# SHI-Labs/SH-GAN

Measured on AMD Instinct MI355X. Metric: generator images/sec, higher is better.
Workload: dtype f32

## Files before the change

include/shgan_hip.h:

```cpp
#ifndef SHGAN_HIP_H
#define SHGAN_HIP_H
#include <stddef.h>
#include <stdint.h>
#ifdef __cplusplus
extern "C" {
#endif

#define SHG_OK 0
#define SHG_ERR_ARG (-1)
#define SHG_ERR_LAUNCH (-2)
#define SHG_ERR_UNSUPPORTED (-3)

int shg_abi_version(void);
const char* shg_last_error(void);
int shg_device_info(int dev, char* buf, int buflen);

int shg_upfirdn2d_out_size(int H, int W, int fh, int fw, int upx, int upy, int downx, int downy, int padx0, int padx1,
                           int pady0, int pady1, int* OH, int* OW);
int shg_upfirdn2d_f32(const float* x, const float* f, float* y, int N, int C, int H, int W, int fh, int fw, int upx, int upy,
                      int downx, int downy, int padx0, int padx1, int pady0, int pady1, int flip, float gain, void* stream);
int shg_upfirdn2d_strided(const void* x, const float* f, void* y, int dtype, int N, int C, int H, int W, const long* x_strides,
                          const long* y_strides, int fh, int fw, long f_stride_y, long f_stride_x, int upx, int upy, int downx, int downy,
                          int padx0, int padx1, int pady0, int pady1, int flip, float gain, void* stream);
int shg_upfirdn2d_epilogue_f32(const float* x, const float* f, float* y, int N, int C, int H, int W, int fh, int fw, int upx,
// ... 15 lines not shown
int shg_sum_partials_f32(const float* part, float* out, int N, int B, int K, void* stream);
int shg_scale_cast_f32_f16(const void* src, void* dst, long n, float gain, int to_half, void* stream);
int shg_planes_to_image_f32(const float* mid, const float* bias, float* y, int N, int C, int H, int W, int lo, int OH, int OW,
                            void* stream);

int shg_conv_weight_prep_f32(const float* w, float* wt, float* wscale, float* wsq, int O, int I, int KH, int KW, int OP,
                             int demod, float gain, int flip, void* stream);
int shg_conv2d_f32(const float* x, const float* wt, float* y, int NB, int I, int O, int OP, int H, int W, int kh, int kw,
                   int mode, int pad, int wgroups, long wstride, const float* in_scale, const float* out_scale,
                   const float* bias, const float* noise, int noise_mode, float noise_strength, int act, float alpha, float gain,
                   float clamp, const float* residual, int out_mode, void* workspace, size_t ws_bytes, void* stream);
size_t shg_conv2d_workspace_bytes(int NB, int I, int O, int H, int W, int kh, int kw, int mode, int pad, int wgroups);
int shg_conv_wino_chunk(void);
int shg_conv_weight_prep_wino_f32(const float* w, const float* wscale, float* wu, int O, int I, int OP, int flip, void* stream);
int shg_conv2d_wino_f32(const float* x, const float* wu, float* y, int NB, int I, int O, int OP, int H, int W,
                        const float* in_scale, const float* out_scale, const float* bias, const float* noise, int noise_mode,
                        float noise_strength, int act, float alpha, float gain, float clamp, const float* residual, void* stream);
size_t shg_conv2d_wino_workspace_bytes(int NB, int I, int O, int OP, int H, int W);
int shg_conv2d_wino_ws_f32(const float* x, const float* wu, float* y, int NB, int I, int O, int OP, int H, int W,
                           const float* in_scale, const float* out_scale, const float* bias, const float* noise, int noise_mode,
                           float noise_strength, int act, float alpha, float gain, float clamp, const float* residual, void* workspace,
                           size_t ws_bytes, void* stream);
long shg_conv_wino4_weight_elems(int OP, int I);
int shg_conv_weight_prep_wino4_f32(const float* w, const float* wscale, float* wu, int O, int I, int OP, int flip, void* stream);
int shg_conv2d_wino4_supported(int NB, int I, int O, int H, int W);
int shg_conv2d_wino4_f32(const float* x, const float* wu, float* y, int NB, int I, int O, int OP, int H, int W,
                         const float* in_scale, const float* out_scale, const float* bias, const float* noise, int noise_mode,
                         float noise_strength, int act, float alpha, float gain, float clamp, const float* residual, void* stream);
size_t shg_conv2d_wino4_workspace_bytes(int NB, int I, int O, int OP, int H, int W);
int shg_conv2d_wino4_ws_f32(const float* x, const float* wu, float* y, int NB, int I, int O, int OP, int H, int W,
                            const float* in_scale, const float* out_scale, const float* bias, const float* noise, int noise_mode,
                            float noise_strength, int act, float alpha, float gain, float clamp, const float* residual, void* workspace,
                            size_t ws_bytes, void* stream);
int shg_upfir_planar_f32(const float* mid, const float* f, float* y, int N, int C, int H, int W, int flip, float gain,
                         const float* scale, const float* bias, const float* noise, int noise_mode, float noise_strength,
                         int act, float alpha, float act_gain, float clamp, const float* residual, void* stream);
int shg_upfir_planar_sep_supported(int H, int W);
int shg_upfir_planar_sep_f32(const float* mid, const float* taps_host, float* y, int N, int C, int H, int W, int flip, float gain,
                             const float* scale, const float* bias, const float* noise, int noise_mode, float noise_strength,
                             int act, float alpha, float act_gain, float clamp, const float* residual, void* stream);
int shg_conv_weight_prep_up_poly_f32(const float* w, const float* wscale, float* wu_a, float* wu_b, int O, int I, int OP, int flip,
                                     void* stream);
int shg_conv2d_up_poly_supported(int NB, int I, int O, int H, int W);
int shg_conv2d_up_poly_f32(const float* x, const float* wt, const float* wu_a, const float* wu_b, float* y, int NB, int I, int O,
                           int OP, int H, int W, const float* in_scale, void* stream);
size_t shg_conv2d_up_poly_workspace_bytes(int NB, int I, int O, int OP, int H, int W);
int shg_conv2d_up_poly_ws_f32(const float* x, const float* wt, const float* wu_a, const float* wu_b, float* y, int NB, int I, int O,
                              int OP, int H, int W, const float* in_scale, void* workspace, size_t ws_bytes, void* stream);
int shg_fir_down_planar_f32(const float* x, const float* f, float* y, int N, int C, int H, int W, int PP, int flip, float gain,
                            void* stream);
int shg_fir_pad2_sep_supported(int H, int W, int PP);
int shg_fir_pad2_sep_f32(const float* x, const float* taps_host, float* y, int N, int C, int H, int W, int PP, int flip, float gain,
                         void* stream);
int shg_fir_resample2_sep_supported(int H, int W, int up);
int shg_fir_resample2_sep_f32(const float* x, const float* taps_host, float* y, int N, int C, int H, int W, int up, int flip, float gain,
                              void* stream);
int shg_conv_weight_prep_down_poly_f32(const float* w, const float* wscale, float* wu_a, float* wu_b, int O, int I, int OP, int flip,
                                       void* stream);
int shg_conv2d_down_poly_supported(int NB, int I, int O, int OH, int OW);
int shg_conv2d_down_poly_f32(const float* xp, const float* wu_a, const float* wu_b, float* y, int NB, int I, int O, int OP, int OH,
                             int OW, int PP, const float* in_scale, const float* bias, int act, float alpha, float gain,
                             float clamp, const float* residual, void* stream);
int shg_conv1x1_thin_in_f32(const float* x, const float* w, const float* bias, float* y, int N, int I, int O, int HW, float wgain,
                            int act, float alpha, float gain, float clamp, void* stream);
int shg_torgb_f32(const float* x, const float* w, const float* styles, const float* bias, const float* base_up, const float* f,
                  float* y, int N, int I, int O, int H, int W, void* stream);
// ... 169 lines not shown
```

sh-gan_amd/_lib.py:

```python
import ctypes
import os

import torch

_HERE = os.path.dirname(os.path.abspath(__file__))
LIB_PATH = os.path.join(_HERE, 'lib', 'libshgan_hip.so')
ABI_VERSION = 40

c_fp = ctypes.c_void_p
c_i = ctypes.c_int
c_f = ctypes.c_float
c_l = ctypes.c_long
c_pp = ctypes.POINTER(ctypes.c_void_p)



class DenseGroup(ctypes.Structure):
    _fields_ = [('x1', c_fp), ('x2', c_fp), ('w', c_fp), ('b', c_fp), ('y', c_fp),
                ('ld1', c_i), ('ld2', c_i), ('K1', c_i), ('K2', c_i), ('O', c_i), ('ldy', c_i),
                ('wgain', c_f), ('bgain', c_f)]


class StyleGroup(ctypes.Structure):
    _fields_ = [('styles', c_fp), ('wsq', c_fp), ('s_out', c_fp), ('dcoef', c_fp),
# ... 5 lines not shown
        (n, c_i) for n in ('I', 'H', 'W', 'x_ctot', 'x_coff', 'O', 'kh', 'kw', 'sh', 'sw', 'ph', 'pw', 'OH', 'OW', 'y_ctot', 'y_coff', 'splitk')]


_SIGS = {
    'shg_abi_version': [],
    'shg_device_info': [c_i, ctypes.c_char_p, c_i],
    'shg_upfirdn2d_out_size': [c_i] * 12 + [ctypes.POINTER(c_i), ctypes.POINTER(c_i)],
    'shg_upfirdn2d_f32': [c_fp, c_fp, c_fp] + [c_i] * 15 + [c_f, c_fp],
    'shg_upfirdn2d_strided': [c_fp, c_fp, c_fp, c_i, c_i, c_i, c_i, c_i, ctypes.POINTER(c_l), ctypes.POINTER(c_l), c_i, c_i, c_l, c_l] + [c_i] * 9
                             + [c_f, c_fp],
    'shg_upfirdn2d_epilogue_f32': [c_fp, c_fp, c_fp] + [c_i] * 15 + [c_f, c_fp, c_fp, c_fp, c_i, c_f, c_i, c_f, c_f, c_f, c_fp, c_fp],
    'shg_bias_act_f32': [c_fp, c_fp, c_fp, c_fp, c_fp, c_i, c_f, c_fp, c_i, c_i, c_i, c_i, c_f, c_f, c_f, c_fp],
    'shg_fma_f32': [c_fp, c_fp, c_fp, c_fp, c_l, c_fp],
    'shg_fma_bcast': [c_fp, c_fp, c_fp, c_fp, c_i] + [ctypes.POINTER(c_l)] * 4 + [c_i, c_fp],
    'shg_mul_reduce': [c_fp, c_fp, c_fp, c_i, c_i] + [ctypes.POINTER(c_l)] * 3 + [c_i, c_i, c_fp],
    'shg_scale_channels_f32': [c_fp, c_fp, c_fp, c_i, c_i, c_fp],
    'shg_sum_partials_f32': [c_fp, c_fp, c_i, c_i, c_i, c_fp],
    'shg_scale_cast_f32_f16': [c_fp, c_fp, c_l, c_f, c_i, c_fp],
    'shg_planes_to_image_f32': [c_fp, c_fp, c_fp, c_i, c_i, c_i, c_i, c_i, c_i, c_i, c_fp],
    'shg_conv_weight_prep_f32': [c_fp, c_fp, c_fp, c_fp, c_i, c_i, c_i, c_i, c_i, c_i, c_f, c_i, c_fp],
    'shg_conv2d_f32': [c_fp, c_fp, c_fp] + [c_i] * 11 + [c_l, c_fp, c_fp, c_fp, c_fp, c_i, c_f, c_i, c_f, c_f, c_f, c_fp, c_i,
                       c_fp, ctypes.c_size_t, c_fp],
    'shg_conv2d_workspace_bytes': [c_i] * 10,
    'shg_conv_wino_chunk': [],
    'shg_conv_weight_prep_wino_f32': [c_fp, c_fp, c_fp, c_i, c_i, c_i, c_i, c_fp],
    'shg_conv2d_wino_f32': [c_fp, c_fp, c_fp] + [c_i] * 6 + [c_fp, c_fp, c_fp, c_fp, c_i, c_f, c_i, c_f, c_f, c_f, c_fp, c_fp],
    'shg_conv2d_wino_ws_f32': [c_fp, c_fp, c_fp] + [c_i] * 6 + [c_fp, c_fp, c_fp, c_fp, c_i, c_f, c_i, c_f, c_f, c_f, c_fp, c_fp, ctypes.c_size_t, c_fp],
    'shg_conv2d_wino_workspace_bytes': [c_i] * 6,
    'shg_conv_wino4_weight_elems': [c_i, c_i],
    'shg_conv_weight_prep_wino4_f32': [c_fp, c_fp, c_fp, c_i, c_i, c_i, c_i, c_fp],
    'shg_conv2d_wino4_supported': [c_i] * 5,
    'shg_conv2d_wino4_f32': [c_fp, c_fp, c_fp] + [c_i] * 6 + [c_fp, c_fp, c_fp, c_fp, c_i, c_f, c_i, c_f, c_f, c_f, c_fp, c_fp],
    'shg_conv2d_wino4_ws_f32': [c_fp, c_fp, c_fp] + [c_i] * 6 + [c_fp, c_fp, c_fp, c_fp, c_i, c_f, c_i, c_f, c_f, c_f, c_fp, c_fp, ctypes.c_size_t, c_fp],
    'shg_conv2d_wino4_workspace_bytes': [c_i] * 6,
    'shg_upfir_planar_f32': [c_fp, c_fp, c_fp, c_i, c_i, c_i, c_i, c_i, c_f, c_fp, c_fp, c_fp, c_i, c_f, c_i, c_f, c_f, c_f, c_fp, c_fp],
    'shg_upfir_planar_sep_supported': [c_i, c_i],
    'shg_upfir_planar_sep_f32': [c_fp, ctypes.POINTER(c_f), c_fp, c_i, c_i, c_i, c_i, c_i, c_f, c_fp, c_fp, c_fp, c_i, c_f, c_i, c_f, c_f, c_f, c_fp, c_fp],
    'shg_conv1x1_thin_in_f32': [c_fp, c_fp, c_fp, c_fp, c_i, c_i, c_i, c_i, c_f, c_i, c_f, c_f, c_f, c_fp],
    'shg_torgb_f32': [c_fp, c_fp, c_fp, c_fp, c_fp, c_fp, c_fp, c_i, c_i, c_i, c_i, c_i, c_fp],
    'shg_dense_f32': [c_fp, c_fp, c_fp, c_fp, c_i, c_i, c_i, c_i, c_i, c_f, c_f, c_i, c_f, c_f, c_f, c_fp],
    'shg_demod_weight_f32': [c_fp, c_fp, c_fp, c_fp, c_i, c_i, c_i, c_i, c_fp],
    'shg_demod_weight_backward_f32': [c_fp, c_fp, c_fp, c_fp, c_fp, c_i, c_i, c_i, c_fp],
    'shg_style_factors_f32': [c_fp, c_fp, c_fp, c_fp, c_fp, c_i, c_i, c_i, c_i, c_fp],
    'shg_style_factors_backward_f32': [c_fp, c_fp, c_fp, c_fp, c_fp, c_fp, c_fp, c_fp, c_fp, c_i, c_i, c_i, c_i, c_fp],
    'shg_matmul_nn_f32': [c_fp, c_fp, c_fp, c_i, c_i, c_i, c_i, c_i, c_f, c_fp],
    'shg_matmul_tn_f32': [c_fp, c_fp, c_fp, c_fp, c_i, c_i, c_i, c_i, c_i, c_f, c_f, c_fp],
    'shg_normalize_2nd_moment_f32': [c_fp, c_fp, c_i, c_i, c_f, c_fp],
    'shg_modconv_style_prep_f32': [c_fp, c_i, c_fp, c_fp, c_fp, c_i, c_i, c_i, c_i, c_i, c_f, c_fp],
    'shg_dense_grouped_f32': [ctypes.POINTER(DenseGroup), c_i, c_i, c_fp],
    'shg_modconv_style_prep_grouped_f32': [ctypes.POINTER(StyleGroup), c_i, c_i, c_fp],
    'shg_shu_rfft2_shift_f32': [c_fp, c_l, c_fp, c_i, c_i, c_fp],
    'shg_bias_act_backward_f32': [c_fp, c_fp, c_fp, c_l, c_i, c_f, c_f, c_f, c_fp],
    'shg_conv2d_wgrad_workspace_bytes': [c_i] * 7,
    'shg_conv2d_wgrad_f32': [c_fp, c_fp, c_fp] + [c_i] * 11 + [c_fp, ctypes.c_size_t, c_fp],
    'shg_conv2d_wgrad_wino_supported': [c_i] * 8,
    'shg_conv2d_wgrad_wino_workspace_bytes': [c_i] * 5,
    'shg_conv2d_wgrad_wino_f32': [c_fp, c_fp, c_fp] + [c_i] * 5 + [c_fp, ctypes.c_size_t, c_fp],
    'shg_shu_spectral_f32': [c_fp] * 6 + [c_i] * 4 + [c_fp],
    'shg_shu_split_irfft2_f32': [c_fp, c_fp, c_pp, c_pp, ctypes.POINTER(c_l), c_i, c_i, c_i, c_i, c_fp],
    'shg_shu_split_adjoint_f32': [c_pp, ctypes.POINTER(c_l), c_pp, c_fp, c_i, c_i, c_fp],
    'shg_shu_rfft2_shift_n_f32': [c_fp, c_l, c_fp, c_i, c_i, c_i, c_fp],
    'shg_shu_spectral_n_f32': [c_fp] * 6 + [c_i] * 4 + [c_fp],
    'shg_shu_split_irfft2_n_f32': [c_fp, c_fp, c_pp, c_pp, ctypes.POINTER(c_l), c_i, c_i, c_i, c_i, c_i, ctypes.POINTER(c_i), c_i, c_fp],
    'shg_shu_split_adjoint_n_f32': [c_pp, ctypes.POINTER(c_l), c_pp, c_fp, c_i, c_i, c_i, ctypes.POINTER(c_i), c_i, c_fp],
    'shg_composite_u8': [c_fp, c_fp, c_fp, c_i, c_i, c_i, c_fp],
    'shg_assemble_input_f32': [c_fp, c_fp, c_fp, c_i, c_i, c_i, c_fp],
# ... 124 lines not shown
```

sh-gan_amd/csrc/conv_wino4.hip:

```cpp
#include "wino_common.h"
#include <stdlib.h>
#include <type_traits>

__device__ __attribute__((aligned(16))) float shg_wino4_zeros[64];

namespace wino4 {
constexpr int KC = 8, BO = 64, BT = 32, NPOS = 36, NW = 8, NT = NW * 64, NUNIT = 2 * NPOS;
constexpr int V_SZ = NPOS * KC * BT;
template <int TY, int TX>
struct Tile {
    static_assert(TY * TX == BT, "32 blocks per tile");
    static constexpr int PH = 4 * TY + 2, PW = 4 * TX + 8, PW4 = PW / 4, PATCH4 = PH * PW4;
    static constexpr int NPIECE = (PATCH4 + 63) / 64, RP = NPIECE * 256, R_SZ = KC * RP;
};
static_assert(2 * V_SZ >= NPOS * 16 * 32, "epilogue exchange buffer lives in the V region");
}

template <class T>
__device__ __forceinline__ void wino4_bt(const T (&d)[6], T (&o)[6]) {
    const T a = d[4] - 4.f * d[2], b = d[3] - 4.f * d[1], c = d[4] - d[2], e = 2.f * (d[3] - d[1]);
    o[0] = 4.f * d[0] - 5.f * d[2] + d[4];
    o[1] = a + b; o[2] = a - b;
    o[3] = c + e; o[4] = c - e;
    o[5] = 4.f * d[1] - 5.f * d[3] + d[5];
}
__device__ __forceinline__ void wino4_at(const float (&m)[6], float (&o)[4]) {
    float s12 = m[1] + m[2], d12 = m[1] - m[2], s34 = m[3] + m[4], d34 = m[3] - m[4];
    shg_opaque(s12); shg_opaque(d12); shg_opaque(s34); shg_opaque(d34);
    o[0] = m[0] + s12 + s34;
    o[1] = d12 + 2.f * d34;
    o[2] = s12 + 4.f * s34;
    o[3] = d12 + 8.f * d34 + m[5];
}

template <int TY, int TX>
__global__ __launch_bounds__(512, 2) void conv_wino4_kernel(const WinoParams p) {
    using namespace wino4;
    using T = Tile<TY, TX>;
    constexpr int PW = T::PW, PW4 = T::PW4, PATCH4 = T::PATCH4, RP = T::RP, R_SZ = T::R_SZ, NPIECE = T::NPIECE;
    __shared__ __attribute__((aligned(16))) float Vl[2 * V_SZ];
    __shared__ __attribute__((aligned(16))) float Rl[2 * R_SZ];

    const int tid = threadIdx.x;
    const int lane = tid & 63, wave = __builtin_amdgcn_readfirstlane(tid >> 6);
    const int l31 = lane & 31, half = lane >> 5;

    const int nwork = p.n_ttiles * p.n_otiles;
    const int work = shg_xcd_remap(blockIdx.x, nwork);
    const int otile = work / p.n_ttiles;
    const int ttile = work - otile * p.n_ttiles;
    const int txb = ttile % p.tiles_x;
    const int tyb = (ttile / p.tiles_x) % p.tiles_y;
    const int n = ttile / (p.tiles_x * p.tiles_y);
    const int oy0 = tyb * (4 * TY), ox0 = txb * (4 * TX);
    const int o0 = otile * BO;
    const int HW = p.H * p.W;
    const int c0 = blockIdx.y * p.cps, nch = min(p.cps, p.nchunk - c0), iend = min(p.I, (c0 + nch) * KC);

    const bool xformer = wave < 4;
    int roff[NPIECE];
#pragma unroll
    for (int j = 0; j < NPIECE; ++j) {
        const int q = j * 64 + lane;
        const int py = q / PW4, p4 = q - py * PW4;
        const int iy = oy0 - 1 + py, ix = ox0 - 4 + 4 * p4;
        const bool ok = q < PATCH4 && iy >= 0 && iy < p.H && ix >= 0 && ix + 3 < p.W;
        roff[j] = ok ? n * p.I * HW + iy * p.W + ix : -1;
    }
    auto dma_piece = [&](int c, int buf, int q, int j) __attribute__((always_inline)) {
        const int k = (wave - 4) * 2 + q;
        const int ch = (c0 + c) * KC + k;
        const bool chok = ch < iend;
        const float* src = (chok && roff[j] >= 0) ? p.x + ((long)roff[j] + (long)ch * HW) : shg_wino4_zeros;
        const unsigned lds = __builtin_amdgcn_readfirstlane(
// ... 23 lines not shown
        const float s1 = __builtin_bit_cast(float, __builtin_amdgcn_readlane(__builtin_bit_cast(int, ca < 64 ? scb[0] : scb[1]), ca & 63));
        return half ? s1 : s0;
    };
    auto tr_read = [&](int r, f32x4 (&w)[3], int buf) __attribute__((always_inline)) {
        const f32x4* rb = reinterpret_cast<const f32x4*>(rbase + buf * R_SZ + r * PW);
#pragma unroll
        for (int q = 0; q < 3; ++q) w[q] = rb[q];
    };
    auto tr_row = [&](int r, const f32x4 (&w)[3], float (&u)[6][6], float sc) __attribute__((always_inline)) {
        const float di[6] = {w[0][3] * sc, w[1][0] * sc, w[1][1] * sc, w[1][2] * sc, w[1][3] * sc, w[2][0] * sc};
        wino4_bt(di, u[r]);
    };
    auto tr_col = [&](int j, const float (&u)[6][6], int buf) __attribute__((always_inline)) {
        float* vb = vbase + buf * V_SZ + j * KC * BT;
        const float di[6] = {u[0][j], u[1][j], u[2][j], u[3][j], u[4][j], u[5][j]};
        float o[6];
        wino4_bt(di, o);
#pragma unroll
        for (int i = 0; i < 6; ++i) vb[i * 6 * KC * BT] = o[i];
    };

    float* Mx = Vl;
    const long plane = (long)p.H * p.W;
    const int o_l = tid >> 5, t_l = tid & 31;
    const int by = t_l / TX, bx = t_l % TX;
    const int oy = oy0 + 4 * by, ox = ox0 + 4 * bx;
    auto body = [&](auto nu_c, auto xf_c) __attribute__((always_inline)) {
        constexpr int NU = decltype(nu_c)::value;
        constexpr bool XF = decltype(xf_c)::value;
        constexpr int NP = NU / 2;
        const int pfirst = XF ? 4 * wave : 16 + 5 * (wave - 4);
        constexpr size_t ustride = (size_t)4 * NUNIT * 64;
        const float* ubase = p.wu + ((size_t)otile * p.nchunk * 4 * NUNIT + 2 * pfirst) * 64 + lane + (size_t)c0 * ustride;
        float ur[4][NU];
        auto load_u = [&](int c, int ks) __attribute__((always_inline)) {
#pragma unroll
            for (int j = 0; j < NU; ++j) ur[ks][j] = ubase[(size_t)c * ustride + (ks * NUNIT + j) * 64];
        };
        f32x16 acc[NU];
        const float* bbase = Vl + (pfirst * KC + half) * BT + l31;

        float b[2][NP];
#pragma unroll
        for (int ks = 0; ks < 3; ++ks) load_u(0, ks);
        if constexpr (!XF) {
            dma_raw(0, 0);
            dma_raw(1, 1);
        }
        __builtin_amdgcn_s_waitcnt(0x0F70);
        __syncthreads();
        if constexpr (XF) {
            f32x4 w[3];
            float u[6][6];
            const float sc = style_of(0);
#pragma unroll
            for (int r = 0; r < 6; ++r) {
                tr_read(r, w, 0);
                tr_row(r, w, u, sc);
            }
#pragma unroll
            for (int j = 0; j < 6; ++j) tr_col(j, u, 0);
        }
        __syncthreads();

        const int last = nch - 1;
        auto fetch = [&](const float* bb, int ks, int pb) __attribute__((always_inline)) {
#pragma unroll
            for (int q = 0; q < NP; ++q) b[pb][q] = bb[(q * KC + ks * 2) * BT];
        };
        auto mma = [&](int ks, int pb, int j) __attribute__((always_inline)) {
            acc[j] = __builtin_amdgcn_mfma_f32_32x32x2f32(ur[ks][j], b[pb][j >> 1], acc[j], 0, 0, 0);
        };
        auto mma_first = [&](int ks, int pb, int j) __attribute__((always_inline)) {
            const f32x16 z = {0.f, 0.f, 0.f, 0.f, 0.f, 0.f, 0.f, 0.f, 0.f, 0.f, 0.f, 0.f, 0.f, 0.f, 0.f, 0.f};
            acc[j] = __builtin_amdgcn_mfma_f32_32x32x2f32(ur[ks][j], b[pb][j >> 1], z, 0, 0, 0);
        };
        auto refill = [&](int c, int ks, int j) __attribute__((always_inline)) {
            ur[ks][j] = ubase[(size_t)c * ustride + (ks * NUNIT + j) * 64];
        };
        auto chunk = [&](auto first_c, int c) __attribute__((always_inline)) {
            constexpr bool FIRST = decltype(first_c)::value;
            const int buf = c & 1;
            const int cn = c < last ? c + 1 : last;
            const float* bb = bbase + buf * V_SZ;
            f32x4 w[2][3];
            float u[6][6];
            float sc = 1.f;
            if constexpr (XF) sc = style_of(cn);
            fetch(bb, 0, 0);
            __builtin_amdgcn_sched_barrier(0);
            constexpr int RFD = 2;
            auto refill_m = [&](int m) __attribute__((always_inline)) {
                if (m / NU == 0) refill(c, 3, m % NU);
                else refill(cn, m / NU - 1, m % NU);
            };
#pragma unroll
            for (int j = 0; j < NU; ++j) {
                if constexpr (!FIRST) mma(3, 1, j);
                if constexpr (!XF) {
                    if (j < 2 * NPIECE) dma_piece(c + 2, buf, j / NPIECE, j % NPIECE);
                }
                if (j >= RFD) refill_m(j - RFD);
                if constexpr (XF) {
                    if (j < 6) tr_read(j, w[j & 1], buf ^ 1);
                    if (j >= 1 && j < 7) tr_row(j - 1, w[(j - 1) & 1], u, sc);
                }
                __builtin_amdgcn_sched_barrier(0);
            }
#pragma unroll
            for (int ks = 0; ks < 3; ++ks) {
                fetch(bb, ks + 1, (ks + 1) & 1);
                __builtin_amdgcn_sched_barrier(0);
#pragma unroll
                for (int j = 0; j < NU; ++j) {
                    if (FIRST && ks == 0) mma_first(ks, ks & 1, j);
                    else mma(ks, ks & 1, j);
                    refill_m((ks + 1) * NU + j - RFD);
                    if constexpr (XF) {
                        if (ks == 0 && j < 6) tr_col(j, u, buf ^ 1);
                    }
                    __builtin_amdgcn_sched_barrier(0);
                }
            }
#pragma unroll
            for (int m = 4 * NU - RFD; m < 4 * NU; ++m) refill_m(m);
            if constexpr (!XF) asm volatile("s_waitcnt vmcnt(%0)" ::"n"(4 * NU - 2 * NPIECE + 1 + RFD) : "memory");
            asm volatile("s_waitcnt lgkmcnt(0)" ::: "memory");
            __builtin_amdgcn_s_barrier();
            asm volatile("" ::: "memory");
        };
        chunk(std::true_type{}, 0);
        for (int c = 1; c < nch; ++c) chunk(std::false_type{}, c);
#pragma unroll
        for (int j = 0; j < NU; ++j) mma(3, 1, j);

        const bool col_ok = oy < p.H && ox < p.W;
        const int oxc = ox < p.W ? ox : 0;
        long rowoff[4];
    #pragma unroll
        for (int i = 0; i < 4; ++i) rowoff[i] = (long)(oy + i < p.H ? oy + i : p.H - 1) * p.W + oxc;
        f32x4 nz[4];
        {
            const float* np_ = p.noise_mode ? p.noise + (p.noise_mode == 2 ? (long)n * plane : 0) : shg_wino4_zeros;
    #pragma unroll
            for (int i = 0; i < 4; ++i) nz[i] = *reinterpret_cast<const f32x4*>(np_ + (p.noise_mode ? rowoff[i] : 0)) * p.noise_strength;
        }
        const ShgAct actc = shg_act_make(p.act, p.alpha, p.gain, p.clamp);
        struct TailOps { float osc, bs; f32x4 rs[4]; };
        auto tail_load = [&](int pass, TailOps& t) __attribute__((always_inline)) {
            const int oo = o0 + (pass >> 1) * 32 + 16 * (pass & 1) + o_l;
            const int oc = oo < p.O ? oo : p.O - 1;
            t.osc = p.out_scale ? p.out_scale[(long)n * p.O + oc] : 1.f;
            t.bs = p.bias ? p.bias[oc] : 0.f;
            const float* rp = p.residual ? p.residual + ((long)n * p.O + oc) * plane : shg_wino4_zeros;
    #pragma unroll
            for (int i = 0; i < 4; ++i) t.rs[i] = *reinterpret_cast<const f32x4*>(rp + (p.residual ? rowoff[i] : 0));
        };
        auto finish = [&](int pass, TailOps& t) __attribute__((always_inline)) {
            const int ob = pass >> 1, h = pass & 1;
            const int o = o0 + ob * 32 + 16 * h + o_l;
            float tmp[6][4];
    #pragma unroll
            for (int r = 0; r < 6; ++r) {
                float m[6], a4[4];
    #pragma unroll
                for (int cc = 0; cc < 6; ++cc) m[cc] = Mx[((r * 6 + cc) * 16 + o_l) * 32 + t_l];
                wino4_at(m, a4);
// ... 17 lines not shown
                    out[i][k] = v + t.rs[i][k];
                }
            }
            if (pass < 3) tail_load(pass + 1, t);
            if (o < p.O && col_ok) {
                float* yp = p.y + blockIdx.y * p.part_stride + ((long)n * p.O + o) * plane;
    #pragma unroll
                for (int i = 0; i < 4; ++i)
                    if (oy + i < p.H) *reinterpret_cast<f32x4*>(yp + rowoff[i]) = out[i];
            }
        };

        TailOps tops;
        tail_load(0, tops);
#pragma unroll
        for (int pass = 0; pass < 4; ++pass) {
            const int ob = pass >> 1, h = pass & 1;
#pragma unroll
            for (int q = 0; q < NP; ++q) {
#pragma unroll
                for (int rr = 0; rr < 8; ++rr) {
                    const int r = 8 * h + rr;
                    const int lr = (r & 3) + 8 * ((r >> 2) & 1) + 4 * half;
                    Mx[((pfirst + q) * 16 + lr) * 32 + l31] = acc[2 * q + ob][r];
                }
            }
            __syncthreads();
            finish(pass, tops);
            if (pass < 3) __syncthreads();
        }
    };
    if (xformer) body(std::integral_constant<int, 8>{}, std::true_type{});
    else body(std::integral_constant<int, 10>{}, std::false_type{});
}

__global__ __launch_bounds__(256) void wino4_weight_kernel(const float* w, const float* scale, float* wu, int O, int I, int OP,
                                                           int nchunk, int flip) {
    constexpr int KC = wino4::KC;
    const long e = (long)blockIdx.x * 256 + threadIdx.x;
    const long total = (long)OP * nchunk * KC;
    if (e >= total) return;
    const int o = (int)(e % OP);
    const int i = (int)(e / OP);
    float g[3][3];
#pragma unroll
    for (int t = 0; t < 9; ++t) {
        const int tt = flip ? 8 - t : t;
        g[t / 3][t % 3] = (o < O && i < I) ? w[((long)o * I + i) * 9 + tt] * scale[o] : 0.f;
    }
    float gg[6][3];
#pragma unroll
    for (int cc = 0; cc < 3; ++cc) {
        const float a = g[0][cc], b = g[1][cc], c = g[2][cc];
        gg[0][cc] = a * 0.25f;
        gg[1][cc] = (-a - b - c) * (1.f / 6.f);
        gg[2][cc] = (-a + b - c) * (1.f / 6.f);
        gg[3][cc] = a * (1.f / 24.f) + b * (1.f / 12.f) + c * (1.f / 6.f);
        gg[4][cc] = a * (1.f / 24.f) - b * (1.f / 12.f) + c * (1.f / 6.f);
        gg[5][cc] = c;
    }
    const int k = i % KC, chunk = i / KC;
    const int ln = (k & 1) * 32 + (o & 31), ks = k >> 1, obk = (o & 63) >> 5;
    float* base = wu + ((size_t)(o >> 6) * nchunk + chunk) * (4 * wino4::NUNIT * 64);
#pragma unroll
    for (int r = 0; r < 6; ++r) {
        const float a = gg[r][0], b = gg[r][1], c = gg[r][2];
        const float row[6] = {a * 0.25f, (-a - b - c) * (1.f / 6.f), (-a + b - c) * (1.f / 6.f),
                              a * (1.f / 24.f) + b * (1.f / 12.f) + c * (1.f / 6.f), a * (1.f / 24.f) - b * (1.f / 12.f) + c * (1.f / 6.f), c};
#pragma unroll
        for (int cc = 0; cc < 6; ++cc) {
            const int u = (r * 6 + cc) * 2 + obk;
            base[((size_t)ks * wino4::NUNIT + u) * 64 + ln] = row[cc];
        }
    }
}

extern "C" long shg_conv_wino4_weight_elems(int OP, int I) {
    return (long)(OP / 64) * shg_cdiv(I, wino4::KC) * 4 * wino4::NUNIT * 64;
}

extern "C" int shg_conv_weight_prep_wino4_f32(const float* w, const float* wscale, float* wu, int O, int I, int OP, int flip,
                                              void* stream) {
    SHG_CHECK_ARG(w && wscale && wu, "weight_prep_wino4: null pointer");
    SHG_CHECK_ARG(O >= 1 && I >= 1 && OP % 64 == 0 && OP >= O, "weight_prep_wino4: bad shape");
    const int nchunk = shg_cdiv(I, wino4::KC);
    const long total = (long)OP * nchunk * wino4::KC;
    hipLaunchKernelGGL(wino4_weight_kernel, dim3(shg_cdiv(total, 256)), dim3(256), 0, (hipStream_t)stream, w, wscale, wu, O, I, OP,
                       nchunk, flip);
    SHG_CHECK_LAUNCH();
    return SHG_OK;
}

extern "C" int shg_conv2d_wino4_supported(int NB, int I, int O, int H, int W) {
    return (H >= 16 && W >= 32 && W % 4 == 0 && I <= 128 * wino4::KC && NB >= 1 && O >= 1) ? 1 : 0;
}

static int wino4_plan(WinoParams& p, int NB, int I, int OP, int H, int W) {
    const int shape = (W >= 256 && H >= 4) ? 2 : ((W >= 128 && H >= 8) ? 1 : 0);
    p.tiles_x = shg_cdiv(W, 32 << shape); p.tiles_y = shg_cdiv(H, 16 >> shape);
    p.n_ttiles = p.tiles_x * p.tiles_y * NB; p.n_otiles = OP / 64; p.nchunk = shg_cdiv(I, wino4::KC);
    return shape;
}

extern "C" size_t shg_conv2d_wino4_workspace_bytes(int NB, int I, int O, int OP, int H, int W) {
    if (NB < 1 || I < 1 || O < 1 || OP < 64 || H < 1 || W < 1) return 0;
    WinoParams p{};
    wino4_plan(p, NB, I, OP, H, W);
    return shg_wino_split_bytes((long)p.n_ttiles * p.n_otiles, p.nchunk, (size_t)NB * O * H * W * sizeof(float));
}

extern "C" int shg_conv2d_wino4_ws_f32(const float* x, const float* wu, float* y, int NB, int I, int O, int OP, int H, int W,
                                       const float* in_scale, const float* out_scale, const float* bias, const float* noise,
                                       int noise_mode, float noise_strength, int act, float alpha, float gain, float clamp,
                                       const float* residual, void* workspace, size_t ws_bytes, void* stream) {
    SHG_CHECK_ARG(x && wu && y, "conv2d_wino4: null pointer");
    SHG_CHECK_ARG(shg_conv2d_wino4_supported(NB, I, O, H, W), "conv2d_wino4: unsupported geometry (use shg_conv2d_wino_f32)");
    SHG_CHECK_ARG(OP % 64 == 0 && OP >= O, "conv2d_wino4: OP must be a multiple of 64 and >= O");
    SHG_CHECK_ARG((long)NB * I * H * W < 2147483647L && (long)NB * O * H * W < 2147483647L, "conv2d_wino4: tensor too large");
    SHG_CHECK_ARG(((shg_addr(x) | shg_addr(y) | shg_addr(noise) | shg_addr(residual)) & 15) == 0, "conv2d_wino4: x / y / noise / residual must be 16-byte aligned");
    WinoParams p = shg_wino_params(x, wu, y, NB, I, O, OP, H, W, in_scale, out_scale, bias, noise, noise_mode, noise_strength, act, alpha, gain, clamp, residual);
    const int shape = wino4_plan(p, NB, I, OP, H, W);
    const int ks = shg_wino_split(p, workspace, ws_bytes, shg_addr(workspace));
    const dim3 grid(p.n_ttiles * p.n_otiles, ks);
    if (shape == 2) hipLaunchKernelGGL((conv_wino4_kernel<1, 32>), grid, dim3(wino4::NT), 0, (hipStream_t)stream, p);
    else if (shape == 1) hipLaunchKernelGGL((conv_wino4_kernel<2, 16>), grid, dim3(wino4::NT), 0, (hipStream_t)stream, p);
    else hipLaunchKernelGGL((conv_wino4_kernel<4, 8>), grid, dim3(wino4::NT), 0, (hipStream_t)stream, p);
    SHG_CHECK_LAUNCH();
    if (ks > 1) {
        shg_launch_wino_split_reduce((const float*)workspace, y, ks, NB, O, H, W, out_scale, bias, noise_mode ? noise : nullptr, noise ? noise_mode : 0,
                                     noise_strength, act, alpha, gain, clamp, residual, (hipStream_t)stream);
        SHG_CHECK_LAUNCH();
    }
    return SHG_OK;
}

extern "C" int shg_conv2d_wino4_f32(const float* x, const float* wu, float* y, int NB, int I, int O, int OP, int H, int W,
                                    const float* in_scale, const float* out_scale, const float* bias, const float* noise,
                                    int noise_mode, float noise_strength, int act, float alpha, float gain, float clamp,
                                    const float* residual, void* stream) {
    return shg_conv2d_wino4_ws_f32(x, wu, y, NB, I, O, OP, H, W, in_scale, out_scale, bias, noise, noise_mode, noise_strength, act, alpha, gain, clamp,
                                   residual, nullptr, 0, stream);
}
```

sh-gan_amd/kernels.py:

```python
import contextlib
import ctypes
import math

import torch

from . import _lib
from ._lib import check

SQRT2 = math.sqrt(2.0)
_NULLCTX = contextlib.nullcontext()


class _Launch:
    __slots__ = ('dev', 'keep', '_ctx')

    def __init__(self):
        self.dev = None
        self.keep = []
        self._ctx = None

    def _own(self, t, name):
        if self.dev is None:
            self.dev = t.device
        elif t.device != self.dev:
# ... 535 lines not shown
            w, ws = L.req(self._w, 'w'), L.req(self._wscale, 'wscale')
            self.wu4 = L.new((int(_lib.get_lib().shg_conv_wino4_weight_elems(self.op, self.i)),))
            with L:
                check(_lib.get_lib().shg_conv_weight_prep_wino4_f32(_ptr(w), _ptr(ws), _ptr(self.wu4), self.o, self.i, self.op,
                                                                    int(bool(self._flip)), L.stream()), 'conv_weight_prep_wino4')
        return self.wu4


def conv_weight_prep(w, demod=False, gain=1.0, flip=False, groups=1):
    L = _Launch()
    w = L.req(w, 'w')
    o_all, i, kh, kw = w.shape
    o = o_all // groups
    op = (o + 63) // 64 * 64
    kk = kh * kw
    ip = (i + 31) // 32 * 32
    wt = L.new((groups, ip * kk * op))
    wsq = L.new((groups, i * op)) if demod else None
    wscale = L.new((o,))
    lib = _lib.get_lib()
    with L:
        for g in range(groups):
            wg = w[g * o:(g + 1) * o]
            check(lib.shg_conv_weight_prep_f32(_ptr(wg), _ptr(wt[g]), _ptr(wscale), _ptr(wsq[g]) if demod else None, o, i, kh, kw,
                                               op, int(bool(demod)), float(gain), int(bool(flip)), L.stream()), 'conv_weight_prep')
    keep = groups == 1 and kh == 3 and kw == 3
    return PreppedWeight(wt, wsq, o, i, op, kh, kw, groups, w=w if keep else None, wscale=wscale if keep else None, flip=flip)


WINO = True
WINO_MIN = 16
WINO4 = True
WINO4_MIN = 32
WINO_SPLIT = True
UP_POLY = True
DOWN_POLY = True

MODE_SAME, MODE_DOWN2, MODE_UP2T = 0, 1, 2
_CONV_CLASS = {MODE_SAME: 'conv_mfma_s1', MODE_DOWN2: 'conv_mfma_s2', MODE_UP2T: 'conv_mfma_up'}


def _wino_workspace(L, bytes_fn, *shape):
    ws_bytes = int(bytes_fn(*shape)) if WINO_SPLIT else 0
    return (L.new((ws_bytes // 4,)) if ws_bytes else None), ws_bytes


def conv2d(x, pw, mode=MODE_SAME, pad=0, in_scale=None, out_scale=None, bias=None, noise=None, noise_strength=1.0,
           act=False, gain=1.0, alpha=0.2, act_gain=SQRT2, clamp=256.0, residual=None, planar=False):
    L = _Launch()
    x = L.req(x, 'x')
    nb, i, h, w = x.shape
    if i != pw.i:
        raise _lib.ShgError(f'conv2d: x has {i} channels, weights expect {pw.i}')
    L.view(pw.wt, 'weights')
    if mode == MODE_SAME:
        oh, ow = h + 2 * pad - pw.kh + 1, w + 2 * pad - pw.kw + 1
    elif mode == MODE_DOWN2:
        oh, ow = (h + 2 * pad - pw.kh) // 2 + 1, (w + 2 * pad - pw.kw) // 2 + 1
    else:
        oh, ow = 2 * h + 1, 2 * w + 1
    lib = _lib.get_lib()
    if mode == MODE_UP2T and planar:
        y = L.new((4, nb, pw.o, h + 1, w + 1))
    else:
        y = L.new((nb, pw.o, oh, ow))
    noise, nmode = _noise_args(L, noise, nb)
    a, al, g, cl = _act_args(act, gain, alpha, act_gain, clamp)
    residual = L.req(residual, 'residual')
    in_scale, out_scale, bias = L.req(in_scale, 'in_scale'), L.req(out_scale, 'out_scale'), L.req(bias, 'bias')
    if residual is not None and tuple(residual.shape) != tuple(y.shape):
        raise _lib.ShgError('conv2d: residual shape mismatch')
    tail_al = (_addr(noise) or 0) | (_addr(residual) or 0)
    if (WINO and mode == MODE_SAME and pad == 1 and pw.kh == 3 and pw.kw == 3 and pw.groups == 1 and h >= WINO_MIN and w >= WINO_MIN
            and w % 4 == 0 and x.data_ptr() % 16 == 0 and tail_al % 8 == 0 and i <= 1024 and (pw.wu is not None or pw._w is not None)):
        direct = 2.0 * nb * pw.o * i * 9 * oh * ow
        if WINO4 and h >= WINO4_MIN and tail_al % 16 == 0 and lib.shg_conv2d_wino4_supported(nb, i, pw.o, h, w):
            wu = pw.wino4()
            executed = 2.0 * nb * pw.o * i * 36.0 * ((h + 3) // 4) * ((w + 3) // 4)
            ws, ws_bytes = _wino_workspace(L, lib.shg_conv2d_wino4_workspace_bytes, nb, i, pw.o, pw.op, h, w)
            with _timed(L, 'conv_wino4', direct, executed):
                check(lib.shg_conv2d_wino4_ws_f32(
                    _ptr(x), _ptr(wu), _ptr(y), nb, i, pw.o, pw.op, h, w, _ptr(in_scale), _ptr(out_scale), _ptr(bias), _ptr(noise),
                    nmode, float(noise_strength), a, al, g, cl, _ptr(residual), _ptr(ws), ws_bytes, L.stream()), 'conv2d_wino4')
            return y
        wu = pw.wino()
        ws, ws_bytes = _wino_workspace(L, lib.shg_conv2d_wino_workspace_bytes, nb, i, pw.o, pw.op, h, w)
        with _timed(L, 'conv_wino', direct, direct * 16.0 / 36.0):
            check(lib.shg_conv2d_wino_ws_f32(
                _ptr(x), _ptr(wu), _ptr(y), nb, i, pw.o, pw.op, h, w, _ptr(in_scale), _ptr(out_scale), _ptr(bias), _ptr(noise), nmode,
                float(noise_strength), a, al, g, cl, _ptr(residual), _ptr(ws), ws_bytes, L.stream()), 'conv2d_wino')
        return y
    if (UP_POLY and mode == MODE_UP2T and planar and pw.groups == 1 and pw._w is not None and out_scale is None and bias is None
            and noise is None and residual is None and not act and gain == 1.0 and x.data_ptr() % 16 == 0
            and lib.shg_conv2d_up_poly_supported(nb, i, pw.o, h, w)):
        wa, wb = pw.up_poly()
        nba, nbb = ((h + 1 + 2) // 3) * ((w + 1 + 2) // 3), (h // 2) * (w // 2)
        executed = 2.0 * nb * pw.o * i * (16.0 * (nba + nbb) + h + w)
        ws, ws_bytes = _wino_workspace(L, lib.shg_conv2d_up_poly_workspace_bytes, nb, i, pw.o, pw.op, h, w)
        with _timed(L, 'conv_poly_up', 2.0 * nb * pw.o * i * 9 * h * w, executed):
            check(lib.shg_conv2d_up_poly_ws_f32(_ptr(x), _ptr(pw.wt), _ptr(wa), _ptr(wb), _ptr(y), nb, i, pw.o, pw.op, h, w,
                                                _ptr(in_scale), _ptr(ws), ws_bytes, L.stream()), 'conv2d_up_poly')
        return y
    ws, ws_bytes = None, 0
    if mode != MODE_UP2T or planar:
        ws_bytes = int(lib.shg_conv2d_workspace_bytes(nb, i, pw.o, h, w, pw.kh, pw.kw, mode, pad, pw.groups))
        if ws_bytes:
            ws = L.new((ws_bytes // 4,))
    pix = (h * w) if mode == MODE_UP2T else (oh * ow)
    with _timed(L, _CONV_CLASS[mode] if pw.kh == 3 else 'conv_mfma_1x1', 2.0 * nb * pw.o * i * pw.kh * pw.kw * pix):
        check(lib.shg_conv2d_f32(
            _ptr(x), _ptr(pw.wt), _ptr(y), nb, i, pw.o, pw.op, h, w, pw.kh, pw.kw, mode, pad, pw.groups, pw.wt.shape[1],
            _ptr(in_scale), _ptr(out_scale), _ptr(bias), _ptr(noise), nmode, float(noise_strength), a, al, g, cl, _ptr(residual),
            1 if planar else 0, _ptr(ws), ws_bytes, L.stream()), 'conv2d')
    return y


# ... 426 lines not shown
```

Measured before the change: 839.1.

## Stage Winograd-4 U weights through an LDS ring via direct global-to-LDS loads

Adds a variant of the wino4 conv kernel in which each wave streams its transformed-weight (U) slices into a double-buffered LDS ring using global_load_lds_dwordx4. Mfma operands are then read from LDS one step ahead instead of being held in four register sets. The aim is to cut VGPR pressure and overlap weight fetch with the MFMA loop. The planner also now avoids the widest 1x32 tile shape for layers with I>=64, so those layers land on the tile shapes that can use the ring. A route argument and a Python knob allow forcing the register or LDS path. The hand-tuned vmcnt wait counts are fragile and add LDS usage.

```diff
diff --git a/include/shgan_hip.h b/include/shgan_hip.h
--- a/include/shgan_hip.h
+++ b/include/shgan_hip.h
@@ -71,6 +71,10 @@
                             const float* in_scale, const float* out_scale, const float* bias, const float* noise, int noise_mode,
                             float noise_strength, int act, float alpha, float gain, float clamp, const float* residual, void* workspace,
                             size_t ws_bytes, void* stream);
+int shg_conv2d_wino4_route_f32(const float* x, const float* wu, float* y, int NB, int I, int O, int OP, int H, int W,
+                               const float* in_scale, const float* out_scale, const float* bias, const float* noise, int noise_mode,
+                               float noise_strength, int act, float alpha, float gain, float clamp, const float* residual, int route,
+                               void* workspace, size_t ws_bytes, void* stream);
 int shg_upfir_planar_f32(const float* mid, const float* f, float* y, int N, int C, int H, int W, int flip, float gain,
                          const float* scale, const float* bias, const float* noise, int noise_mode, float noise_strength,
                          int act, float alpha, float act_gain, float clamp, const float* residual, void* stream);
diff --git a/sh-gan_amd/_lib.py b/sh-gan_amd/_lib.py
--- a/sh-gan_amd/_lib.py
+++ b/sh-gan_amd/_lib.py
@@ -61,6 +61,7 @@
     'shg_conv2d_wino4_supported': [c_i] * 5,
     'shg_conv2d_wino4_f32': [c_fp, c_fp, c_fp] + [c_i] * 6 + [c_fp, c_fp, c_fp, c_fp, c_i, c_f, c_i, c_f, c_f, c_f, c_fp, c_fp],
     'shg_conv2d_wino4_ws_f32': [c_fp, c_fp, c_fp] + [c_i] * 6 + [c_fp, c_fp, c_fp, c_fp, c_i, c_f, c_i, c_f, c_f, c_f, c_fp, c_fp, ctypes.c_size_t, c_fp],
+    'shg_conv2d_wino4_route_f32': [c_fp, c_fp, c_fp] + [c_i] * 6 + [c_fp, c_fp, c_fp, c_fp, c_i, c_f, c_i, c_f, c_f, c_f, c_fp, c_i, c_fp, ctypes.c_size_t, c_fp],
     'shg_conv2d_wino4_workspace_bytes': [c_i] * 6,
     'shg_upfir_planar_f32': [c_fp, c_fp, c_fp, c_i, c_i, c_i, c_i, c_i, c_f, c_fp, c_fp, c_fp, c_i, c_f, c_i, c_f, c_f, c_f, c_fp, c_fp],
     'shg_upfir_planar_sep_supported': [c_i, c_i],
diff --git a/sh-gan_amd/csrc/conv_wino4.hip b/sh-gan_amd/csrc/conv_wino4.hip
--- a/sh-gan_amd/csrc/conv_wino4.hip
+++ b/sh-gan_amd/csrc/conv_wino4.hip
@@ -14,6 +14,11 @@
     static constexpr int NPIECE = (PATCH4 + 63) / 64, RP = NPIECE * 256, R_SZ = KC * RP;
 };
 static_assert(2 * V_SZ >= NPOS * 16 * 32, "epilogue exchange buffer lives in the V region");
+constexpr int UR_XF = 2 * 8 * 64, UR_FE = 2 * 12 * 64, UR_SZ = 4 * UR_XF + 4 * UR_FE;
+constexpr int LDS_BYTES = 163840;
+template <int TY, int TX> constexpr bool uring_fits() { return (2 * V_SZ + 2 * Tile<TY, TX>::R_SZ + UR_SZ) * 4 <= LDS_BYTES; }
+template <int TY, int TX> constexpr bool uring_default() { return uring_fits<TY, TX>(); }
+constexpr int URING_WIDE_MIN_I = 64;
 }
 
 template <class T>
@@ -33,13 +38,15 @@
     o[3] = d12 + 8.f * d34 + m[5];
 }
 
-template <int TY, int TX>
-__global__ __launch_bounds__(512, 2) void conv_wino4_kernel(const WinoParams p) {
+template <int TY, int TX, bool URING>
+__device__ __forceinline__ void conv_wino4_body(const WinoParams& p) {
     using namespace wino4;
     using T = Tile<TY, TX>;
     constexpr int PW = T::PW, PW4 = T::PW4, PATCH4 = T::PATCH4, RP = T::RP, R_SZ = T::R_SZ, NPIECE = T::NPIECE;
+    static_assert(!URING || (uring_fits<TY, TX>() && 2 * NPIECE == 6), "the U ring needs 40 960 B beside V and the windows; its load counts assume six window pieces");
     __shared__ __attribute__((aligned(16))) float Vl[2 * V_SZ];
     __shared__ __attribute__((aligned(16))) float Rl[2 * R_SZ];
+    __shared__ __attribute__((aligned(16))) float Ul[URING ? UR_SZ : 4];
 
     const int tid = threadIdx.x;
     const int lane = tid & 63, wave = __builtin_amdgcn_readfirstlane(tid >> 6);
@@ -129,17 +136,57 @@
         const int pfirst = XF ? 4 * wave : 16 + 5 * (wave - 4);
         constexpr size_t ustride = (size_t)4 * NUNIT * 64;
         const float* ubase = p.wu + ((size_t)otile * p.nchunk * 4 * NUNIT + 2 * pfirst) * 64 + lane + (size_t)c0 * ustride;
-        float ur[4][NU];
+        float ur[URING ? 1 : 4][NU];
         auto load_u = [&](int c, int ks) __attribute__((always_inline)) {
 #pragma unroll
             for (int j = 0; j < NU; ++j) ur[ks][j] = ubase[(size_t)c * ustride + (ks * NUNIT + j) * 64];
+        };
+        constexpr int SU = XF ? 8 : 12, NPC = XF ? 2 : 3;
+        float* uring = Ul + (XF ? wave * UR_XF : 4 * UR_XF + (wave - 4) * UR_FE);
+        const float* usrc = ubase - lane + lane * 4;
+        const float* usrc2 = ubase - lane + 512 + (lane & 31) * 4;
+        auto u_piece = [&](int c, int ks, int slot, int q) __attribute__((always_inline)) {
+            const float* src = (q < 2 ? usrc + q * 256 : usrc2) + ((size_t)c * ustride + ks * NUNIT * 64);
+            const unsigned lds = __builtin_amdgcn_readfirstlane(
+                (unsigned)(size_t)(__attribute__((address_space(3))) void*)(uring + (slot * SU + q * 4) * 64));
+            asm volatile("s_mov_b32 m0, %0\n\ts_nop 0\n\tglobal_load_lds_dwordx4 %1, off" ::"s"(lds), "v"(src) : "m0", "memory");
+        };
+        auto u_wait = [&](int n) __attribute__((always_inline)) {
+            switch (n) {
+            case 1: asm volatile("s_waitcnt vmcnt(1)" ::: "memory"); break;
+            case 2: asm volatile("s_waitcnt vmcnt(2)" ::: "memory"); break;
+            case 3: asm volatile("s_waitcnt vmcnt(3)" ::: "memory"); break;
+            case 4: asm volatile("s_waitcnt vmcnt(4)" ::: "memory"); break;
+            case 5: asm volatile("s_waitcnt vmcnt(5)" ::: "memory"); break;
+            case 8: asm volatile("s_waitcnt vmcnt(8)" ::: "memory"); break;
+            case 9: asm volatile("s_waitcnt vmcnt(9)" ::: "memory"); break;
+            default: asm volatile("s_waitcnt vmcnt(0)" ::: "memory"); break;
+            }
+        };
+        auto u_step = [&](bool first, int c, int cn, int G, int j) __attribute__((always_inline)) {
+            if constexpr (XF) {
+                if (j == 2 || j == 6) u_wait(1);
+            } else {
+                if (j == 0) u_wait(3 + (G == 1 ? 6 : 0) + (G == 0 ? 1 : 0));
+                if (j == 2) u_wait(2 + (G == 1 ? 2 : 0) + (G == 0 ? 3 : 0));
+                if (j == 6) u_wait(2 + (G == 0 ? 6 : 0));
+            }
+            if (j >= 2) ur[0][j - 2] = uring[((G & 1) * SU + j - 2) * 64 + lane];
+            else if (!first) ur[0][NU - 2 + j] = uring[(((G + 1) & 1) * SU + NU - 2 + j) * 64 + lane];
+            if (j == 3 || j == 7 || (!XF && j == 9))
+                u_piece(G < 3 ? c : cn, (G + 1) & 3, (G + 1) & 1, j == 3 ? 0 : (j == 7 ? 1 : 2));
         };
         f32x16 acc[NU];
         const float* bbase = Vl + (pfirst * KC + half) * BT + l31;
 
         float b[2][NP];
-#pragma unroll
-        for (int ks = 0; ks < 3; ++ks) load_u(0, ks);
+        if constexpr (URING) {
+#pragma unroll
+            for (int q = 0; q < NPC; ++q) u_piece(0, 0, 0, q);
+        } else {
+#pragma unroll
+            for (int ks = 0; ks < 3; ++ks) load_u(0, ks);
+        }
         if constexpr (!XF) {
             dma_raw(0, 0);
             dma_raw(1, 1);
@@ -166,11 +213,11 @@
             for (int q = 0; q < NP; ++q) b[pb][q] = bb[(q * KC + ks * 2) * BT];
         };
         auto mma = [&](int ks, int pb, int j) __attribute__((always_inline)) {
-            acc[j] = __builtin_amdgcn_mfma_f32_32x32x2f32(ur[ks][j], b[pb][j >> 1], acc[j], 0, 0, 0);
+            acc[j] = __builtin_amdgcn_mfma_f32_32x32x2f32(ur[URING ? 0 : ks][j], b[pb][j >> 1], acc[j], 0, 0, 0);
         };
         auto mma_first = [&](int ks, int pb, int j) __attribute__((always_inline)) {
             const f32x16 z = {0.f, 0.f, 0.f, 0.f, 0.f, 0.f, 0.f, 0.f, 0.f, 0.f, 0.f, 0.f, 0.f, 0.f, 0.f, 0.f};
-            acc[j] = __builtin_amdgcn_mfma_f32_32x32x2f32(ur[ks][j], b[pb][j >> 1], z, 0, 0, 0);
+            acc[j] = __builtin_amdgcn_mfma_f32_32x32x2f32(ur[URING ? 0 : ks][j], b[pb][j >> 1], z, 0, 0, 0);
         };
         auto refill = [&](int c, int ks, int j) __attribute__((always_inline)) {
             ur[ks][j] = ubase[(size_t)c * ustride + (ks * NUNIT + j) * 64];
@@ -197,7 +244,8 @@
                 if constexpr (!XF) {
                     if (j < 2 * NPIECE) dma_piece(c + 2, buf, j / NPIECE, j % NPIECE);
                 }
-                if (j >= RFD) refill_m(j - RFD);
+                if constexpr (URING) u_step(FIRST, c, cn, 0, j);
+                else if (j >= RFD) refill_m(j - RFD);
                 if constexpr (XF) {
                     if (j < 6) tr_read(j, w[j & 1], buf ^ 1);
                     if (j >= 1 && j < 7) tr_row(j - 1, w[(j - 1) & 1], u, sc);
@@ -212,16 +260,19 @@
                 for (int j = 0; j < NU; ++j) {
                     if (FIRST && ks == 0) mma_first(ks, ks & 1, j);
                     else mma(ks, ks & 1, j);
-                    refill_m((ks + 1) * NU + j - RFD);
+                    if constexpr (URING) u_step(false, c, cn, ks + 1, j);
+                    else refill_m((ks + 1) * NU + j - RFD);
                     if constexpr (XF) {
                         if (ks == 0 && j < 6) tr_col(j, u, buf ^ 1);
                     }
                     __builtin_amdgcn_sched_barrier(0);
                 }
             }
-#pragma unroll
-            for (int m = 4 * NU - RFD; m < 4 * NU; ++m) refill_m(m);
-            if constexpr (!XF) asm volatile("s_waitcnt vmcnt(%0)" ::"n"(4 * NU - 2 * NPIECE + 1 + RFD) : "memory");
+            if constexpr (!URING) {
+#pragma unroll
+                for (int m = 4 * NU - RFD; m < 4 * NU; ++m) refill_m(m);
+            }
+            if constexpr (!XF) asm volatile("s_waitcnt vmcnt(%0)" ::"n"(URING ? 2 + 3 * NPC : 4 * NU - 2 * NPIECE + 1 + RFD) : "memory");
             asm volatile("s_waitcnt lgkmcnt(0)" ::: "memory");
             __builtin_amdgcn_s_barrier();
             asm volatile("" ::: "memory");
@@ -229,7 +280,15 @@
         chunk(std::true_type{}, 0);
         for (int c = 1; c < nch; ++c) chunk(std::false_type{}, c);
 #pragma unroll
-        for (int j = 0; j < NU; ++j) mma(3, 1, j);
+        for (int j = 0; j < NU; ++j) {
+            mma(3, 1, j);
+            if constexpr (URING) {
+                if (!XF && j == 0) u_wait(3);
+                if (j < 2) ur[0][NU - 2 + j] = uring[(SU + NU - 2 + j) * 64 + lane];
+                __builtin_amdgcn_sched_barrier(0);
+            }
+        }
+        if constexpr (URING) asm volatile("s_waitcnt vmcnt(0)" ::: "memory");
 
         const bool col_ok = oy < p.H && ox < p.W;
         const int oxc = ox < p.W ? ox : 0;
@@ -313,6 +372,15 @@
     };
     if (xformer) body(std::integral_constant<int, 8>{}, std::true_type{});
     else body(std::integral_constant<int, 10>{}, std::false_type{});
+}
+
+template <int TY, int TX>
+__global__ __launch_bounds__(512, 2) void conv_wino4_kernel(const WinoParams p) {
+    conv_wino4_body<TY, TX, wino4::uring_default<TY, TX>()>(p);
+}
+template <int TY, int TX>
+__global__ __launch_bounds__(512, 2) void conv_wino4_alt_kernel(const WinoParams p) {
+    conv_wino4_body<TY, TX, !wino4::uring_default<TY, TX>()>(p);
 }
 
 __global__ __launch_bounds__(256) void wino4_weight_kernel(const float* w, const float* scale, float* wu, int O, int I, int OP,
@@ -376,8 +444,9 @@
     return (H >= 16 && W >= 32 && W % 4 == 0 && I <= 128 * wino4::KC && NB >= 1 && O >= 1) ? 1 : 0;
 }
 
-static int wino4_plan(WinoParams& p, int NB, int I, int OP, int H, int W) {
-    const int shape = (W >= 256 && H >= 4) ? 2 : ((W >= 128 && H >= 8) ? 1 : 0);
+static int wino4_plan(WinoParams& p, int NB, int I, int OP, int H, int W, int route = 0) {
+    const bool narrow = route == 3 || (route == 0 && I >= wino4::URING_WIDE_MIN_I);
+    const int shape = (W >= 256 && H >= 4 && !(narrow && H >= 8)) ? 2 : ((W >= 128 && H >= 8) ? 1 : 0);
     p.tiles_x = shg_cdiv(W, 32 << shape); p.tiles_y = shg_cdiv(H, 16 >> shape);
     p.n_ttiles = p.tiles_x * p.tiles_y * NB; p.n_otiles = OP / 64; p.nchunk = shg_cdiv(I, wino4::KC);
     return shape;
@@ -390,22 +459,34 @@
     return shg_wino_split_bytes((long)p.n_ttiles * p.n_otiles, p.nchunk, (size_t)NB * O * H * W * sizeof(float));
 }
 
-extern "C" int shg_conv2d_wino4_ws_f32(const float* x, const float* wu, float* y, int NB, int I, int O, int OP, int H, int W,
-                                       const float* in_scale, const float* out_scale, const float* bias, const float* noise,
-                                       int noise_mode, float noise_strength, int act, float alpha, float gain, float clamp,
-                                       const float* residual, void* workspace, size_t ws_bytes, void* stream) {
+template <int TY, int TX>
+static void wino4_launch(const WinoParams& p, dim3 grid, bool uring, hipStream_t s) {
+    if constexpr (wino4::uring_fits<TY, TX>()) {
+        if (uring != wino4::uring_default<TY, TX>()) {
+            hipLaunchKernelGGL((conv_wino4_alt_kernel<TY, TX>), grid, dim3(wino4::NT), 0, s, p);
+            return;
+        }
+    }
+    hipLaunchKernelGGL((conv_wino4_kernel<TY, TX>), grid, dim3(wino4::NT), 0, s, p);
+}
+
+extern "C" int shg_conv2d_wino4_route_f32(const float* x, const float* wu, float* y, int NB, int I, int O, int OP, int H, int W,
+                                          const float* in_scale, const float* out_scale, const float* bias, const float* noise,
+                                          int noise_mode, float noise_strength, int act, float alpha, float gain, float clamp,
+                                          const float* residual, int route, void* workspace, size_t ws_bytes, void* stream) {
+    SHG_CHECK_ARG(route >= 0 && route <= 3, "conv2d_wino4: route must be 0..3");
     SHG_CHECK_ARG(x && wu && y, "conv2d_wino4: null pointer");
     SHG_CHECK_ARG(shg_conv2d_wino4_supported(NB, I, O, H, W), "conv2d_wino4: unsupported geometry (use shg_conv2d_wino_f32)");
     SHG_CHECK_ARG(OP % 64 == 0 && OP >= O, "conv2d_wino4: OP must be a multiple of 64 and >= O");
     SHG_CHECK_ARG((long)NB * I * H * W < 2147483647L && (long)NB * O * H * W < 2147483647L, "conv2d_wino4: tensor too large");
     SHG_CHECK_ARG(((shg_addr(x) | shg_addr(y) | shg_addr(noise) | shg_addr(residual)) & 15) == 0, "conv2d_wino4: x / y / noise / residual must be 16-byte aligned");
     WinoParams p = shg_wino_params(x, wu, y, NB, I, O, OP, H, W, in_scale, out_scale, bias, noise, noise_mode, noise_strength, act, alpha, gain, clamp, residual);
-    const int shape = wino4_plan(p, NB, I, OP, H, W);
+    const int shape = wino4_plan(p, NB, I, OP, H, W, route);
     const int ks = shg_wino_split(p, workspace, ws_bytes, shg_addr(workspace));
     const dim3 grid(p.n_ttiles * p.n_otiles, ks);
-    if (shape == 2) hipLaunchKernelGGL((conv_wino4_kernel<1, 32>), grid, dim3(wino4::NT), 0, (hipStream_t)stream, p);
-    else if (shape == 1) hipLaunchKernelGGL((conv_wino4_kernel<2, 16>), grid, dim3(wino4::NT), 0, (hipStream_t)stream, p);
-    else hipLaunchKernelGGL((conv_wino4_kernel<4, 8>), grid, dim3(wino4::NT), 0, (hipStream_t)stream, p);
+    if (shape == 2) wino4_launch<1, 32>(p, grid, false, (hipStream_t)stream);
+    else if (shape == 1) wino4_launch<2, 16>(p, grid, route ? route >= 2 : wino4::uring_default<2, 16>(), (hipStream_t)stream);
+    else wino4_launch<4, 8>(p, grid, route ? route >= 2 : wino4::uring_default<4, 8>(), (hipStream_t)stream);
     SHG_CHECK_LAUNCH();
     if (ks > 1) {
         shg_launch_wino_split_reduce((const float*)workspace, y, ks, NB, O, H, W, out_scale, bias, noise_mode ? noise : nullptr, noise ? noise_mode : 0,
@@ -413,6 +494,14 @@
         SHG_CHECK_LAUNCH();
     }
     return SHG_OK;
+}
+
+extern "C" int shg_conv2d_wino4_ws_f32(const float* x, const float* wu, float* y, int NB, int I, int O, int OP, int H, int W,
+                                       const float* in_scale, const float* out_scale, const float* bias, const float* noise,
+                                       int noise_mode, float noise_strength, int act, float alpha, float gain, float clamp,
+                                       const float* residual, void* workspace, size_t ws_bytes, void* stream) {
+    return shg_conv2d_wino4_route_f32(x, wu, y, NB, I, O, OP, H, W, in_scale, out_scale, bias, noise, noise_mode, noise_strength, act, alpha, gain, clamp,
+                                      residual, 0, workspace, ws_bytes, stream);
 }
 
 extern "C" int shg_conv2d_wino4_f32(const float* x, const float* wu, float* y, int NB, int I, int O, int OP, int H, int W,
diff --git a/sh-gan_amd/kernels.py b/sh-gan_amd/kernels.py
--- a/sh-gan_amd/kernels.py
+++ b/sh-gan_amd/kernels.py
@@ -591,6 +591,8 @@
 WINO_MIN = 16
 WINO4 = True
 WINO4_MIN = 32
+WINO4_U = None
+_WINO4_ROUTES = {None: 0, 'reg': 1, 'lds': 2, 'lds_8x64': 3}
 WINO_SPLIT = True
 UP_POLY = True
 DOWN_POLY = True
@@ -638,9 +640,10 @@
             executed = 2.0 * nb * pw.o * i * 36.0 * ((h + 3) // 4) * ((w + 3) // 4)
             ws, ws_bytes = _wino_workspace(L, lib.shg_conv2d_wino4_workspace_bytes, nb, i, pw.o, pw.op, h, w)
             with _timed(L, 'conv_wino4', direct, executed):
-                check(lib.shg_conv2d_wino4_ws_f32(
+                check(lib.shg_conv2d_wino4_route_f32(
                     _ptr(x), _ptr(wu), _ptr(y), nb, i, pw.o, pw.op, h, w, _ptr(in_scale), _ptr(out_scale), _ptr(bias), _ptr(noise),
-                    nmode, float(noise_strength), a, al, g, cl, _ptr(residual), _ptr(ws), ws_bytes, L.stream()), 'conv2d_wino4')
+                    nmode, float(noise_strength), a, al, g, cl, _ptr(residual), _WINO4_ROUTES[WINO4_U], _ptr(ws), ws_bytes, L.stream()),
+                    'conv2d_wino4')
             return y
         wu = pw.wino()
         ws, ws_bytes = _wino_workspace(L, lib.shg_conv2d_wino_workspace_bytes, nb, i, pw.o, pw.op, h, w)
```

New measurement: 848.9 (median of 6 runs). +1.2%, better.
